# ross39/new_bloom_filter_repo

Hardware: AMD Instinct MI355X
Metric: Mpixels/s Bloom insert+query, 1080p residuals (higher is better)
Workload: dtype u64

## Files before the change

new_bloom_filter_repo_amd/csrc/rbf_api.hip:

```cpp
#include "rbf_host.h"
#include "rbf_kernels_noise.h"
#include "rbf_kernels_pack.h"
#include "rbf_rice_host.h"

#include <cmath>

struct MaskArgs {
    const void *frames; FrameLayout l; uint32_t nframes;
    int32_t thr_floor; const int32_t *thr_floors;
    void *masks; uint64_t mask_stride; uint64_t *ones;
    uint32_t channels;
};

static int launch_finish_ones(rbf_ctx *ctx, uint64_t *ones_dev, uint32_t pairs, uint64_t *host_block, uint64_t token,
                              void *clear_a, size_t bytes_a, void *clear_b, size_t bytes_b)
{
    if (clear_a && (((uintptr_t)clear_a | bytes_a) & 15)) { HIP_TRY(hipMemsetAsync(clear_a, 0, bytes_a, ctx->stream)); clear_a = nullptr; bytes_a = 0; }
    if (clear_b && (((uintptr_t)clear_b | bytes_b) & 15)) { HIP_TRY(hipMemsetAsync(clear_b, 0, bytes_b, ctx->stream)); clear_b = nullptr; bytes_b = 0; }
    const uint64_t quads = bytes_a / 16 + bytes_b / 16;
    uint32_t blocks = (uint32_t)((quads + 256 * 4 - 1) / (256 * 4));
    if (blocks < 1) blocks = 1;
    if (blocks > 1024) blocks = 1024;
    hipLaunchKernelGGL(k_finish_ones, dim3(blocks), dim3(256), 0, ctx->stream, ctx->ones_acc.p, ones_dev, pairs, host_block, token,
                       (uint4 *)clear_a, (uint64_t)(bytes_a / 16), (uint4 *)clear_b, (uint64_t)(bytes_b / 16));
// ... 228 lines not shown
}

struct QueryFlags {
    bool image_ready = false;
    bool table_for_next = false;
    bool quiet_passthrough = false;
};

static uint4 *table_to_rewrite(rbf_ctx *ctx, uint64_t n, const Seeds &sd)
{
    const SharedHashTable *sh = ctx->hash_shared;
    if (!sh || sh->n != n || !same_seeds(sh->seeds, sd) || ctx->knobs.no_hash_table || ctx->knobs.no_table_rewrite) return nullptr;
    std::lock_guard<std::mutex> lk(g_hash_mu);
    return sh->refs == 1 ? ctx->hash_tab : nullptr;
}

static int launch_query(rbf_ctx *ctx, const Plan &pl, const BloomBatch &b, const FrameTable &tab, const QueryFlags &flags)
{
    const uint32_t nframes = b.nframes;
    const Seeds sd = to_dev(*b.seeds);
    const uint32_t *filters = (const uint32_t *)b.filters;
    uint64_t stride_words = b.filter_stride / 4;
    if (pl.reads_probe_image()) {
        if (int r = ctx->qimage.reserve((size_t)nframes * pl.image_stride_words * 4)) return r;
        if (!flags.image_ready) {
            const uint32_t bx = (pl.image_stride_words + WG_THREADS - 1) / WG_THREADS;
            hipLaunchKernelGGL(k_probe_image, dim3(bx, nframes), dim3(WG_THREADS), 0, ctx->stream, filters, stride_words, ctx->qimage.p,
                               (uint64_t)pl.image_stride_words);
        }
        filters = ctx->qimage.p;
        stride_words = pl.image_stride_words;
    }
    const uint32_t lds_waves = (uint32_t)((pl.nseg + QL_WAVES - 1) / QL_WAVES);
    uint32_t nactive; uint64_t empty[2];
    LaunchTimer t(ctx, RBF_K_QUERY);
    if (pl.query == QueryKind::LdsTiledF64) {
        const FrameTable stab = query_table_s64(tab, nframes, &nactive, empty);
        if (flags.quiet_passthrough) empty[0] = empty[1] = 0;
        int mode = 0;
        for (uint32_t f = 0; f < nframes; ++f) {
            if (!tab.f[f].m) continue;
            if (tab.f[f].floor_k > 2) mode = 2;
            else if (tab.f[f].floor_k == 0 && mode < 1) mode = 1;
        }
        auto qkern = mode == 2 ? k_query_s64t<2> : mode == 1 ? k_query_s64t<1> : k_query_s64t<0>;
        if (int r = allow_big_lds((const void *)qkern)) return r;
        hipLaunchKernelGGL(qkern, dim3(lds_waves), dim3(QL_THREADS), s64t_lds_bytes(pl.query_tile_words), ctx->stream, b.n, nactive, stab, sd,
                           filters, stride_words, pl.query_tile_words, ctx->seg_cnt.p, pl.nseg, ctx->pass_words.p, empty[0], empty[1]);
    } else if (pl.reads_probe_image()) {
        uint4 *table_out = flags.table_for_next ? table_to_rewrite(ctx, b.n, sd) : nullptr;
        U64Classes cls;
        const FrameTable utab = query_table_u64(tab, nframes, &nactive, &cls, empty);
        if (flags.quiet_passthrough) empty[0] = empty[1] = 0;
        const bool wide = cls.n[3] + cls.n[4] > 0;
        auto kern64 = wide ? k_query_u64w : k_query_u64;
        if (int r = allow_big_lds((const void *)kern64)) return r;
        hipLaunchKernelGGL(kern64, dim3(lds_waves), dim3(QL_THREADS), pl.query_lds_bytes + u64_geo_bytes(nactive), ctx->stream, b.n, nactive,
                           utab, cls, sd, filters, stride_words, pl.fwords_max, ctx->seg_cnt.p, pl.nseg, ctx->pass_words.p, table_out, empty[0],
                           empty[1]);
    } else if (pl.query == QueryKind::LdsWhole) {
        auto kern = pl.double_buffer ? (pl.small_m ? k_query_lds<true, true> : k_query_lds<true, false>)
                                     : (pl.small_m ? k_query_lds<false, true> : k_query_lds<false, false>);
        if (int r = allow_big_lds((const void *)kern)) return r;
        hipLaunchKernelGGL(kern, dim3(lds_waves), dim3(QL_THREADS), pl.query_lds_bytes, ctx->stream, b.n, nframes, tab, sd, filters, stride_words,
                           pl.fwords_max, ctx->seg_cnt.p, pl.nseg, ctx->pass_words.p);
    } else if (pl.query == QueryKind::LdsTiled) {
        auto kern = pl.small_m ? k_query_tiled<true> : k_query_tiled<false>;
        if (int r = allow_big_lds((const void *)kern)) return r;
        hipLaunchKernelGGL(kern, dim3(lds_waves), dim3(QL_THREADS), pl.query_lds_bytes, ctx->stream, b.n, nframes, tab, sd, filters, stride_words,
                           pl.query_tile_words, ctx->seg_cnt.p, pl.nseg, ctx->pass_words.p);
    } else {
        const uint64_t bx = (pl.nseg + WG_WAVES - 1) / WG_WAVES;
        hipLaunchKernelGGL(k_query, dim3((uint32_t)bx, nframes), dim3(WG_THREADS), 0, ctx->stream, b.n, tab, sd, filters, stride_words,
                           ctx->seg_cnt.p, pl.nseg, ctx->pass_words.p);
    }
    return RBF_OK;
}

static int launch_insert_positions(rbf_ctx *ctx, const BloomBatch &b, const FrameTable &itab, const Seeds &sd, bool hashed_positions)
{
    HIP_TRY(hipMemsetAsync(ctx->ins_counters.p, 0, (size_t)b.nframes * 4, ctx->stream));
    const uint64_t groups = (((b.n + 7) >> 3) + IT_STEP_BYTES - 1) / IT_STEP_BYTES;
    uint64_t S1 = (uint64_t)ctx->cus * 4 / (b.nframes ? b.nframes : 1);
    if (S1 > groups / (IP_WAVES * 4)) S1 = groups / (IP_WAVES * 4);
    S1 &= ~7ull;
    if (S1 < 1) S1 = 1;
    if (int r = allow_big_lds((const void *)k_insert_records)) return r;
    LaunchTimer t(ctx, RBF_K_INSERT);
    auto pkern = hashed_positions ? k_insert_positions<true> : k_insert_positions<false>;
    hipLaunchKernelGGL(pkern, dim3((uint32_t)S1, b.nframes), dim3(IP_THREADS), 0, ctx->stream, (const uint8_t *)b.masks, b.mask_stride, b.n, itab,
                       hashed_positions ? nullptr : (const uint4 *)ctx->hash_tab, sd, ctx->ins_records.p, ctx->ins_counters.p);
    return RBF_OK;
}

static bool settle_hash_table(rbf_ctx *ctx, const Plan &pl, const BloomBatch &b, const Seeds &sd)
{
    const bool table_too_big = hash_table_bytes(b.n) > HASH_TABLE_CACHE_BYTES;
    if (table_too_big || (pl.insert_two_phase && ctx->knobs.hash_positions)) {
        if (ctx->hash_shared && (ctx->hash_shared->n != b.n || !same_seeds(ctx->hash_shared->seeds, *b.seeds))) hash_table_release(ctx);
        return true;
    }
    bool built = false;
    if (!hash_table_acquire(ctx, b.n, *b.seeds, &built)) return true;
    if (ctx->knobs.hash_rebuild && !built) launch_hash_table(ctx, b.n, sd, ctx->hash_tab);
    return false;
}

static int insert_fast(rbf_ctx *ctx, const Plan &pl, const BloomBatch &b, const FrameTable &tab, const uint64_t *ones_host, bool stream_once,
                       uint32_t *image)
{
    const uint32_t nframes = b.nframes;
    const Seeds sd = to_dev(*b.seeds);
// ... 1002 lines not shown
```

new_bloom_filter_repo_amd/csrc/rbf_device.h:

```cpp
#pragma once
#include <hip/hip_runtime.h>
#include <stdint.h>

namespace rbf {

constexpr uint64_t P1 = 0x9E3779B185EBCA87ULL;
constexpr uint64_t P2 = 0xC2B2AE3D27D4EB4FULL;
constexpr uint64_t P3 = 0x165667B19E3779F9ULL;
constexpr uint64_t P4 = 0x85EBCA77C2B2AE63ULL;
constexpr uint64_t P5 = 0x27D4EB2F165667C5ULL;

constexpr int WAVE = 64;

struct FrameDev {
    uint32_t m;
    uint32_t floor_k;
    uint64_t T;
    uint64_t M;
};

struct Seeds { uint64_t h1, h2, act; };

constexpr int MAX_BATCH = 128;
struct FrameTable { FrameDev f[MAX_BATCH]; };
// ... 32 lines not shown
    return k;
}

__device__ __forceinline__ uint64_t xxh64_key(const DecKey &k, uint64_t seed)
{
    uint64_t h = seed + P5 + (uint64_t)k.len;
    uint64_t rest;
    uint32_t cnt;
    if (k.len >= 8) {
        uint64_t k1 = k.lo * P2;
        k1 = rotl64(k1, 31) * P1;
        h ^= k1;
        h = rotl64(h, 27) * P1 + P4;
        rest = k.hi; cnt = k.len - 8;
    } else if (k.len >= 4) {
        h ^= (uint64_t)(uint32_t)k.lo * P1;
        h = rotl64(h, 23) * P2 + P3;
        rest = k.lo >> 32; cnt = k.len - 4;
    } else {
        rest = k.lo; cnt = k.len;
    }
    for (uint32_t t = 0; t < cnt; ++t) {
        h ^= (rest & 0xFFu) * P5;
        h = rotl64(h, 11) * P1;
        rest >>= 8;
    }
    h ^= h >> 33; h *= P2;
    h ^= h >> 29; h *= P3;
    h ^= h >> 32;
    return h;
}

struct Hash3 { uint64_t h1, h2, ha; };

template <int LEN>
__device__ __forceinline__ uint64_t xxh64_digits(const uint32_t (&d)[LEN], uint64_t seed)
{
    static_assert(LEN >= 5 && LEN <= 7, "4-byte round + 1..3 byte rounds");
    uint64_t h = seed + P5 + (uint64_t)LEN;
    const uint32_t w = 0x30303030u + d[0] + (d[1] << 8) + (d[2] << 16) + (d[3] << 24);
    h ^= (uint64_t)w * P1;
    h = rotl64(h, 23) * P2 + P3;
#pragma unroll
    for (int t = 4; t < LEN; ++t) {
        h ^= (uint64_t)(0x30u + d[t]) * P5;
        h = rotl64(h, 11) * P1;
    }
    h ^= h >> 33; h *= P2;
    h ^= h >> 29; h *= P3;
    h ^= h >> 32;
    return h;
}

template <int LEN>
__device__ __forceinline__ Hash3 hash3_fixed(uint32_t v, const Seeds &s)
{
    constexpr uint32_t P10[8] = {1u, 10u, 100u, 1000u, 10000u, 100000u, 1000000u, 10000000u};
    uint32_t q[LEN + 1];
#pragma unroll
    for (int k = 0; k <= LEN; ++k) q[k] = k < LEN ? v / P10[k] : 0u;
    uint32_t d[LEN];
#pragma unroll
    for (int k = 0; k < LEN; ++k) d[LEN - 1 - k] = q[k] - 10u * q[k + 1];
    Hash3 r;
    r.h1 = xxh64_digits<LEN>(d, s.h1);
    r.h2 = xxh64_digits<LEN>(d, s.h2);
    r.ha = xxh64_digits<LEN>(d, s.act);
    return r;
}

__device__ __forceinline__ Hash3 hash3_generic(uint32_t v, const Seeds &s)
{
    const DecKey key = make_key(v);
    Hash3 r;
    r.h1 = xxh64_key(key, s.h1);
    r.h2 = xxh64_key(key, s.h2);
    r.ha = xxh64_key(key, s.act);
    return r;
}

__device__ __forceinline__ Hash3 hash3_index(uint32_t v, bool active, const Seeds &s)
{
    const bool in7 = v >= 1000000u && v < 10000000u;
    const bool in6 = v >= 100000u && v < 1000000u;
    const bool in5 = v >= 10000u && v < 100000u;
    if (__all(!active || in7)) return hash3_fixed<7>(active ? v : 1000000u, s);
    if (__all(!active || in6)) return hash3_fixed<6>(active ? v : 100000u, s);
    if (__all(!active || in5)) return hash3_fixed<5>(active ? v : 10000u, s);
    return hash3_generic(active ? v : 0u, s);
}

struct Prefix3 { uint64_t h1, h2, ha; };

template <int LEN>
__device__ __forceinline__ Prefix3 hash3_decade_prefix(uint32_t decade , const Seeds &s)
{
    static_assert(LEN >= 5 && LEN <= 7, "key = decade digits + one more character");
    constexpr uint32_t P10[7] = {1u, 10u, 100u, 1000u, 10000u, 100000u, 1000000u};
    uint32_t q[LEN];
#pragma unroll
    for (int k = 0; k < LEN; ++k) q[k] = k < LEN - 1 ? decade / P10[k] : 0u;
    uint32_t d[LEN - 1];
#pragma unroll
    for (int k = 0; k < LEN - 1; ++k) d[LEN - 2 - k] = q[k] - 10u * q[k + 1];
    const uint64_t lane4 = (uint64_t)(0x30303030u + d[0] + (d[1] << 8) + (d[2] << 16) + (d[3] << 24)) * P1;
    uint64_t h[3] = {s.h1 + P5 + (uint64_t)LEN, s.h2 + P5 + (uint64_t)LEN, s.act + P5 + (uint64_t)LEN};
#pragma unroll
    for (int c = 0; c < 3; ++c) h[c] = rotl64(h[c] ^ lane4, 23) * P2 + P3;
#pragma unroll
    for (int t = 4; t < LEN - 1; ++t) {
        const uint64_t term = (uint64_t)(0x30u + d[t]) * P5;
#pragma unroll
        for (int c = 0; c < 3; ++c) h[c] = rotl64(h[c] ^ term, 11) * P1;
    }
    return Prefix3{h[0], h[1], h[2]};
}

__device__ __forceinline__ uint64_t xxh64_last_byte(uint64_t h, uint64_t term )
{
    h = rotl64(h ^ term, 11) * P1;
    h ^= h >> 33; h *= P2;
    h ^= h >> 29; h *= P3;
    h ^= h >> 32;
    return h;
}

template <int LEN>
__device__ __forceinline__ void hash3_run8_fixed(uint32_t v0, const Seeds &s, uint64_t (&h1)[8], uint64_t (&h2)[8], uint64_t (&ha)[8])
{
    const uint32_t decade = v0 / 10u, r0 = v0 - decade * 10u;
    const Prefix3 a = hash3_decade_prefix<LEN>(decade, s);
    const Prefix3 b = hash3_decade_prefix<LEN>(decade + 1u, s);
#pragma unroll
    for (int j = 0; j < 8; ++j) {
        const uint32_t t = r0 + (uint32_t)j;
        const bool in_b = t >= 10u;
        const uint64_t term = (uint64_t)(0x30u + (in_b ? t - 10u : t)) * P5;
        h1[j] = xxh64_last_byte(in_b ? b.h1 : a.h1, term);
        h2[j] = xxh64_last_byte(in_b ? b.h2 : a.h2, term);
        ha[j] = xxh64_last_byte(in_b ? b.ha : a.ha, term);
    }
}

__device__ __forceinline__ bool hash3_run8(uint32_t v0, uint32_t valid, const Seeds &s, uint64_t (&h1)[8], uint64_t (&h2)[8], uint64_t (&ha)[8])
{
    const bool active = valid != 0u;
    const uint32_t v7 = v0 + 7u;
    const bool in7 = v0 >= 1000000u && v7 < 10000000u;
    const bool in6 = v0 >= 100000u && v7 < 1000000u;
    const bool in5 = v0 >= 10000u && v7 < 100000u;
    if (__all(!active || in7)) { hash3_run8_fixed<7>(active ? v0 : 1000000u, s, h1, h2, ha); return true; }
    if (__all(!active || in6)) { hash3_run8_fixed<6>(active ? v0 : 100000u, s, h1, h2, ha); return true; }
    if (__all(!active || in5)) { hash3_run8_fixed<5>(active ? v0 : 10000u, s, h1, h2, ha); return true; }
    return false;
}

template <int LEN>
__device__ __forceinline__ void hash3_run4_fixed(uint32_t v0, const Seeds &s, uint64_t (&h1)[4], uint64_t (&h2)[4], uint64_t (&ha)[4])
{
    const uint32_t decade = v0 / 10u, r0 = v0 - decade * 10u;
    const Prefix3 a = hash3_decade_prefix<LEN>(decade, s);
    const Prefix3 b = hash3_decade_prefix<LEN>(decade + 1u, s);
#pragma unroll
    for (int j = 0; j < 4; ++j) {
        const uint32_t t = r0 + (uint32_t)j;
        const bool in_b = t >= 10u;
        const uint64_t term = (uint64_t)(0x30u + (in_b ? t - 10u : t)) * P5;
        h1[j] = xxh64_last_byte(in_b ? b.h1 : a.h1, term);
        h2[j] = xxh64_last_byte(in_b ? b.h2 : a.h2, term);
        ha[j] = xxh64_last_byte(in_b ? b.ha : a.ha, term);
    }
}

__device__ __forceinline__ bool hash3_run4(uint32_t v0, uint32_t valid, const Seeds &s, uint64_t (&h1)[4], uint64_t (&h2)[4], uint64_t (&ha)[4])
{
    const bool active = valid != 0u;
    const uint32_t v3 = v0 + 3u;
    const bool in7 = v0 >= 1000000u && v3 < 10000000u;
    const bool in6 = v0 >= 100000u && v3 < 1000000u;
    const bool in5 = v0 >= 10000u && v3 < 100000u;
    if (__all(!active || in7)) { hash3_run4_fixed<7>(active ? v0 : 1000000u, s, h1, h2, ha); return true; }
    if (__all(!active || in6)) { hash3_run4_fixed<6>(active ? v0 : 100000u, s, h1, h2, ha); return true; }
    if (__all(!active || in5)) { hash3_run4_fixed<5>(active ? v0 : 10000u, s, h1, h2, ha); return true; }
    return false;
}

__device__ __forceinline__ uint32_t mod_m(uint64_t h, uint32_t m, uint64_t M)
{
    if (m == 1u) return 0u;
    const uint64_t q = __umul64hi(h, M);
    uint64_t r = h - q * (uint64_t)m;
    if (r >= m) r -= m;
    return (uint32_t)r;
}

struct Probe {
    uint32_t pos;
    uint32_t step;
    bool extra;
};

__device__ __forceinline__ Probe make_probe(uint32_t index, const FrameDev &f, const Seeds &s)
{
    const DecKey key = make_key(index);
    Probe p;
    p.pos = mod_m(xxh64_key(key, s.h1), f.m, f.M);
// ... 13 lines not shown
```

new_bloom_filter_repo_amd/csrc/rbf_kernels_lds.h:

```cpp
#pragma once
#include "rbf_kernels.h"

namespace rbf {

typedef uint32_t nt_u32x4 __attribute__((ext_vector_type(4)));
__device__ __forceinline__ void store_stream(uint4 *p, uint4 v) { const nt_u32x4 x = {v.x, v.y, v.z, v.w}; __builtin_nontemporal_store(x, reinterpret_cast<nt_u32x4 *>(p)); }
__device__ __forceinline__ uint4 load_stream(const uint4 *p) { const nt_u32x4 x = __builtin_nontemporal_load(reinterpret_cast<const nt_u32x4 *>(p)); return make_uint4(x.x, x.y, x.z, x.w); }

constexpr int QL_THREADS = 1024;
constexpr int QL_WAVES = QL_THREADS / WAVE;
constexpr int QL_P = 8;
constexpr int QL_SEG_PIXELS = QL_P * WAVE;

constexpr int IL_THREADS = 1024;
constexpr int IL_WAVES = IL_THREADS / WAVE;
constexpr int IL_QUEUE = 64 + 512;

__device__ __forceinline__ void wave_lds_fence()
{
    __builtin_amdgcn_fence(__ATOMIC_RELEASE, "wavefront");
    __builtin_amdgcn_wave_barrier();
    __builtin_amdgcn_fence(__ATOMIC_ACQUIRE, "wavefront");
}

// ... 625 lines not shown
    if (lane == WAVE - 1) wsum[wave] = incl;
    __syncthreads();
    uint32_t o = start32 + incl - c;
#pragma unroll
    for (int k = 0; k < WG_WAVES; ++k)
        if ((uint32_t)k < wave) o += wsum[k];
    if (w >= nwords) return;
    uint64_t out = 0;
    if (c) {
        const uint32_t d0 = o >> 5, dl = (o + c - 1u) >> 5, r = o & 31u;
        const uint64_t x0 = d0 < witness_stride_words32 ? flip_bytes32(wit[d0]) : 0u;
        const uint64_t x1 = (d0 + 1 <= dl && d0 + 1 < witness_stride_words32) ? flip_bytes32(wit[d0 + 1]) : 0u;
        const uint64_t x2 = (d0 + 2 <= dl && d0 + 2 < witness_stride_words32) ? flip_bytes32(wit[d0 + 2]) : 0u;
        uint64_t win = (x0 | (x1 << 32)) >> r;
        win |= r ? x2 << (64u - r) : 0ull;
        out = (uint64_t)pdep32_lut(lut, (uint32_t)win, p_lo) | ((uint64_t)pdep32_lut(lut, (uint32_t)(win >> c_lo), p_hi) << 32);
    }
    masks[(uint64_t)f * mask_stride_words64 + w] = flip_bytes64(out);
}

}

namespace rbf {

template <typename SAMPLE, int PIXEL_BYTES>
struct LanePixels {
    static constexpr int DW = 16 * PIXEL_BYTES / 4;
    uint32_t d[DW];
    template <bool NT>
    __device__ __forceinline__ void load(const uint8_t *p)
    {
        typedef uint32_t u32x4 __attribute__((ext_vector_type(4)));
        const u32x4 *q = reinterpret_cast<const u32x4 *>(p);
#pragma unroll
        for (int i = 0; i < DW / 4; ++i) {
            const u32x4 v = NT ? __builtin_nontemporal_load(q + i) : q[i];
            d[4 * i] = v.x; d[4 * i + 1] = v.y; d[4 * i + 2] = v.z; d[4 * i + 3] = v.w;
        }
    }
    __device__ __forceinline__ uint32_t luma(int k) const
    {
        const int byte = k * PIXEL_BYTES;
        const uint32_t w = d[byte >> 2];
        if (sizeof(SAMPLE) == 1) return (w >> (8 * (byte & 3))) & 0xFFu;
        return (w >> (8 * (byte & 3))) & 0xFFFFu;
    }
};

template <typename SAMPLE, int PIXEL_BYTES>
__device__ __forceinline__ uint32_t lane_bits_thr0(const LanePixels<SAMPLE, PIXEL_BYTES> &a, const LanePixels<SAMPLE, PIXEL_BYTES> &b, uint32_t one2, uint32_t &count_src)
{
    uint32_t bits = 0;
    if (sizeof(SAMPLE) == 1) {
        constexpr int shift_of_group[4] = {4, 0, 12, 8};
#pragma unroll
        for (int g = 0; g < 4; ++g) {
            uint32_t z;
            if (PIXEL_BYTES == 1) z = a.d[g] ^ b.d[g];
            else {
                const uint32_t x0 = a.d[3 * g] ^ b.d[3 * g], x1 = a.d[3 * g + 1] ^ b.d[3 * g + 1], x2 = a.d[3 * g + 2] ^ b.d[3 * g + 2];
                const uint32_t y = __builtin_amdgcn_perm(x1, x0, 0x00060300u);
                z = __builtin_amdgcn_perm(x2, y, 0x05020100u);
            }
            const uint32_t f = (((z & 0x7F7F7F7Fu) + 0x7F7F7F7Fu) | z) & 0x80808080u;
            bits |= (((f >> 7) * 0x08040201u) >> 24) << shift_of_group[g];
        }
        count_src = bits;
    } else if (PIXEL_BYTES == 2) {
        const uint32_t k7 = 0x7FFF7FFFu;
        uint32_t acc = 0;
#pragma unroll
        for (int s = 0; s < 8; ++s) {
            const int j = s ^ 4;
            const uint32_t t = (a.d[j] ^ b.d[j]) & k7;
            uint32_t g;
            asm("v_pk_min_u16 %0, %1, %2" : "=v"(g) : "v"(t), "v"(one2));
            acc = (acc << 2) | g;
        }
        bits = (acc >> 16) | (acc << 1);
        count_src = acc;
    } else {
        typedef unsigned short h2 __attribute__((ext_vector_type(2)));
#pragma unroll
        for (int j = 0; j < 8; ++j) {
            const h2 t0 = __builtin_bit_cast(h2, a.d[3 * j]) - __builtin_bit_cast(h2, b.d[3 * j]);
            const h2 t1 = __builtin_bit_cast(h2, a.d[3 * j + 1]) - __builtin_bit_cast(h2, b.d[3 * j + 1]);
            const uint32_t d = (__builtin_bit_cast(uint32_t, t0) & 0x0000FFFFu) | (__builtin_bit_cast(uint32_t, t1) & 0xFFFF0000u);
            const uint32_t f = ((d & 0x7FFF7FFFu) + 0x7FFF7FFFu) & 0x80008000u;
            const uint32_t two = ((f >> 14) & 2u) | (f >> 31);
            bits |= two << (((2 * j + 1) ^ 7));
        }
        count_src = bits;
    }
    return bits;
}

template <typename SAMPLE, int PIXEL_BYTES>
__device__ __forceinline__ uint32_t lane_bits_any(const LanePixels<SAMPLE, PIXEL_BYTES> &a, const LanePixels<SAMPLE, PIXEL_BYTES> &b, uint32_t one2, uint32_t &count_src)
{
    static_assert(PIXEL_BYTES == 3 || PIXEL_BYTES == 4 || PIXEL_BYTES == 6 || PIXEL_BYTES == 8, "all-channel masks: 3 or 4 samples of 1 or 2 bytes");
    uint32_t bits = 0;
    if (PIXEL_BYTES == 3) {
        constexpr int shift_of_group[4] = {4, 0, 12, 8};
#pragma unroll
        for (int g = 0; g < 4; ++g) {
            const uint32_t x0 = a.d[3 * g] ^ b.d[3 * g], x1 = a.d[3 * g + 1] ^ b.d[3 * g + 1], x2 = a.d[3 * g + 2] ^ b.d[3 * g + 2];
            const uint32_t s0 = __builtin_amdgcn_perm(x2, __builtin_amdgcn_perm(x1, x0, 0x00060300u), 0x05020100u);
            const uint32_t s1 = __builtin_amdgcn_perm(x2, __builtin_amdgcn_perm(x1, x0, 0x00070401u), 0x06020100u);
            const uint32_t s2 = __builtin_amdgcn_perm(x2, __builtin_amdgcn_perm(x1, x0, 0x00000502u), 0x07040100u);
            const uint32_t z = s0 | s1 | s2;
            const uint32_t f = (((z & 0x7F7F7F7Fu) + 0x7F7F7F7Fu) | z) & 0x80808080u;
            bits |= (((f >> 7) * 0x08040201u) >> 24) << shift_of_group[g];
        }
        count_src = bits;
    } else if (PIXEL_BYTES == 4 || PIXEL_BYTES == 8) {
        constexpr int DPP = PIXEL_BYTES / 4;
#pragma unroll
        for (int k = 0; k < 16; ++k) {
            uint32_t t = a.d[DPP * k] ^ b.d[DPP * k];
// ... 100 lines not shown
```

new_bloom_filter_repo_amd/csrc/rbf_kernels_u64.h:

```cpp
#pragma once
#include "rbf_kernels_s64.h"
#include <algorithm>
#include <cstring>
#include <type_traits>

namespace rbf {

constexpr uint32_t U64_REC_BYTES = 32;
__host__ __device__ constexpr uint32_t u64_geo_bytes(uint32_t nactive) { return (nactive + 1u) * U64_REC_BYTES; }
constexpr int U64_CLASSES = 6;

struct U64Classes { uint32_t n[U64_CLASSES]; };

__host__ inline FrameTable query_table_u64(const FrameTable &tab, uint32_t nframes, uint32_t *nactive, U64Classes *cls, uint64_t (&empty)[2])
{
    FrameTable q;
    memset(&q, 0, sizeof q);
    memset(cls, 0, sizeof *cls);
    empty[0] = empty[1] = 0;
    uint64_t sorted[MAX_BATCH];
    uint32_t coded = 0;
    for (uint32_t f = 0; f < nframes; ++f) {
        if (tab.f[f].m) sorted[coded++] = tab.f[f].T;
        else empty[f >> 6] |= 1ull << (f & 63);
// ... 18 lines not shown
    return q;
}

template <bool ON>
struct RowDmaC {
    const uint8_t *image;
    uint32_t src;
    uint32_t dst_m0;
    uint64_t mask[5];
    bool full;

    __device__ __forceinline__ void issue() const
    {
        uint32_t keep; uint64_t keepx;
        if (full) {
            asm volatile("s_mov_b32 %0, m0\n\t"
                         "s_mov_b32 m0, %1\n\t"
                         "s_nop 0\n\t"
                         "global_load_lds_dwordx4 %2, %3 offset:-2048\n\t"
                         "global_load_lds_dwordx4 %2, %3 offset:-1024\n\t"
                         "global_load_lds_dwordx4 %2, %3\n\t"
                         "global_load_lds_dwordx4 %2, %3 offset:1024\n\t"
                         "global_load_lds_dwordx4 %2, %3 offset:2048\n\t"
                         "s_mov_b32 m0, %0"
                         : "=&s"(keep) : "s"(dst_m0), "v"(src), "s"(image) : "memory");
            return;
        }
        asm volatile("s_mov_b32 %0, m0\n\t"
                     "s_mov_b64 %1, exec\n\t"
                     "s_mov_b32 m0, %2\n\t"
                     "s_mov_b64 exec, %5\n\t"
                     "global_load_lds_dwordx4 %3, %4 offset:-2048\n\t"
                     "s_mov_b64 exec, %6\n\t"
                     "global_load_lds_dwordx4 %3, %4 offset:-1024\n\t"
                     "s_mov_b64 exec, %7\n\t"
                     "global_load_lds_dwordx4 %3, %4\n\t"
                     "s_mov_b64 exec, %8\n\t"
                     "global_load_lds_dwordx4 %3, %4 offset:1024\n\t"
                     "s_mov_b64 exec, %9\n\t"
                     "global_load_lds_dwordx4 %3, %4 offset:2048\n\t"
                     "s_mov_b64 exec, %1\n\t"
                     "s_mov_b32 m0, %0"
                     : "=&s"(keep), "=&s"(keepx)
                     : "s"(dst_m0), "v"(src), "s"(image), "s"(mask[0]), "s"(mask[1]), "s"(mask[2]), "s"(mask[3]), "s"(mask[4])
                     : "memory");
    }
    __device__ __forceinline__ void at(int g)
    {
        if (ON && g == 0) issue();
    }
};


template <bool WIDE>
__device__ __forceinline__ void query_u64_body(
    uint64_t n, uint32_t nactive, const FrameTable &tab, const U64Classes &cls, Seeds seeds,
    const uint32_t *__restrict__ image, uint64_t image_stride_words32, uint32_t fwords_max,
    uint32_t *__restrict__ seg_cnt, uint64_t nseg, uint64_t *__restrict__ pass_words,
    uint4 *__restrict__ table_out, uint64_t empty_lo, uint64_t empty_hi)
{
    extern __shared__ __attribute__((aligned(16))) uint32_t lds[];
    const uint32_t bufwords = ((fwords_max + 3u) & ~3u) + 4u;
    const uint32_t safe_pos = ((fwords_max + 3u) & ~3u) << 5;
    const uint32_t lane = threadIdx.x & 63u, wave = __builtin_amdgcn_readfirstlane(threadIdx.x >> 6);
    const uint32_t seg = blockIdx.x * QL_WAVES + wave;
    const bool live = seg < nseg;
    if (threadIdx.x < 8u) lds[(threadIdx.x >> 2) * bufwords + (bufwords - 4u) + (threadIdx.x & 3u)] = 0u;
    uint4 *geo = reinterpret_cast<uint4 *>(lds + 2u * bufwords);
    uint64_t *tl = reinterpret_cast<uint64_t *>(lds + bufwords);
    FrameDev fd_mine{};
    if (threadIdx.x < 2u * MAX_BATCH) fd_mine = tab.f[threadIdx.x < nactive ? threadIdx.x : 0u];

    static_assert(QL_P == 8, "a lane's verdicts fill one byte");
    double hd1[QL_P], hd2[QL_P];
    uint32_t hl1[QL_P], hl2[QL_P];
    uint32_t rank_lo = 0, rank_hi = 0;
    uint32_t validmask = 0;
    const uint64_t i0 = (uint64_t)seg * QL_SEG_PIXELS + (uint64_t)lane * QL_P;
    {
        uint64_t h1[QL_P], h2[QL_P], ha[QL_P];
#pragma unroll
        for (int it = 0; it < QL_P; ++it) {
            h1[it] = 0; h2[it] = 0; ha[it] = ~0ull;
            if (live && i0 + it < n) validmask |= 1u << it;
        }
        if (!hash3_run8((uint32_t)i0, validmask, seeds, h1, h2, ha)) {
#pragma unroll
            for (int it = 0; it < QL_P; ++it) {
                const bool act = (validmask >> it) & 1u;
                const Hash3 h = hash3_index((uint32_t)(i0 + it), act, seeds);
                h1[it] = h.h1; h2[it] = h.h2; ha[it] = h.ha;
            }
        }
#pragma unroll
        for (int it = 0; it < QL_P; ++it) {
            hd1[it] = (double)h1[it]; hl1[it] = (uint32_t)h1[it];
            hd2[it] = (double)h2[it]; hl2[it] = (uint32_t)h2[it];
        }
        if (table_out && live) hash_table_store8(table_out, n, seg, lane, h1, h2, ha);
        if (threadIdx.x < 2u * MAX_BATCH) {
            const uint32_t t = threadIdx.x;
            tl[t] = t < nactive ? fd_mine.T : ~0ull;
            if (t < nactive) {
                const uint32_t f = fd_mine.floor_k >> 16;
                const uint32_t row = (uint32_t)((uint64_t)f * image_stride_words32 * 4u);
                const uint32_t out_row = (uint32_t)((uint64_t)f * nseg);
                geo[2u * t] = make_uint4(fd_mine.m, (fd_mine.floor_k >> 8) & 0xFFu, (uint32_t)fd_mine.M, (uint32_t)(fd_mine.M >> 32));
                uint32_t *w = reinterpret_cast<uint32_t *>(geo);
                if (t) w[8u * (t - 1u) + 4u] = row;
                if (t + 1u == nactive) w[8u * t + 4u] = row;
                if (t == 0u) w[8u * nactive + 4u] = row;
                w[8u * t + 6u] = fd_mine.floor_k & 0xFFu;
                w[8u * (t + 1u) + 7u] = out_row;
            }
        }
        __syncthreads();
        uint32_t top = 1;
        while (2u * top <= nactive) top *= 2u;
        top = __builtin_amdgcn_readfirstlane(top);
        uint32_t r[QL_P];
#pragma unroll
        for (int it = 0; it < QL_P; ++it) r[it] = 0;
        for (uint32_t step = top; step; step >>= 1) {
#pragma unroll
            for (int it = 0; it < QL_P; ++it) {
                const uint64_t t = tl[r[it] + step - 1u];
                r[it] |= t <= ha[it] ? step : 0u;
            }
        }
        rank_lo = r[0] | (r[1] << 8) | (r[2] << 16) | (r[3] << 24);
        rank_hi = r[4] | (r[5] << 8) | (r[6] << 16) | (r[7] << 24);
    }
    const bool whole_wave = __builtin_amdgcn_readfirstlane((uint32_t)__all(validmask == 0xFFu)) != 0u;
    uint8_t *pass_bytes = reinterpret_cast<uint8_t *>(pass_words);

    for (uint32_t half = 0; half < 2; ++half) {
        uint64_t bits = half ? empty_hi : empty_lo;
        while (bits) {
            const uint32_t g = half * 64u + (uint32_t)__builtin_ctzll(bits);
            bits &= bits - 1;
            if (live && lane == 0) seg_cnt[(uint64_t)g * nseg + seg] = 0;
            if (live) pass_bytes[((uint64_t)g * nseg + seg) * (QL_SEG_PIXELS / 8) + lane] = 0;
        }
    }
    if (nactive == 0) return;

    const uint32_t lds0 = __builtin_amdgcn_readfirstlane(lds_addr_of(lds));
    const uint32_t pitch_bytes = (uint32_t)image_stride_words32 * 4u;
    const uint32_t off0 = wave * 5120u + lane * 16u;
    RowDmaC<true> dm;
    dm.image = reinterpret_cast<const uint8_t *>(image);
#pragma unroll
    for (int i = 0; i < 5; ++i) dm.mask[i] = __ballot(off0 + (uint32_t)i * 1024u + 16u <= pitch_bytes);
    dm.full = dm.mask[4] == ~0ull;
    const uint32_t off0b = off0 + 2048u, wave_dst = wave * 5120u + 2048u;
    const uint32_t buf_sum = lds0 + lds0 + bufwords * 4u;
    uint32_t fbase = vgpr_copy(lds0);
    {
        const uint32_t *w = reinterpret_cast<const uint32_t *>(geo);
        dm.src = w[8u * nactive + 4u] + off0 + 2048u;
        dm.dst_m0 = lds0 + wave * 5120u + 2048u;
        dm.at(0);
    }
    const uint32_t safe_v = vgpr_copy(safe_pos);
    const uint32_t seg_lane = seg * (QL_SEG_PIXELS / 8) + lane;
    uint32_t cnt2 = 0;
    uint32_t row_prev = 0, row_prev2 = 0;
    uint32_t out_row = 0;
    uint32_t out_pb = 0;
    bool out_pending = false, have_two = false;

    auto flush = [&]() {
        if (!out_pending) return;
        if (live) pass_bytes[(out_row << 6) + seg_lane] = (uint8_t)out_pb;
        {
            cnt2 = __builtin_amdgcn_alignbit(__popc(out_pb), cnt2, 16);
            row_prev2 = row_prev; row_prev = out_row;
            if (have_two) {
                const uint32_t tot = wave_sum_to_lane63(cnt2);
                if (live && lane == 63u) {
                    seg_cnt[row_prev2 + seg] = tot & 0xFFFFu;
                    seg_cnt[row_prev + seg] = tot >> 16;
                }
            }
            have_two = !have_two;
        }
    };

    uint32_t j = 0;
    auto frames = [&](auto fk_tag, uint32_t count) {
        constexpr int FK = decltype(fk_tag)::value;
        const uint32_t end = j + count;
        for (; j < end; ++j) {
            const uint4 ga = geo[2u * j], gb = geo[2u * j + 1u];
            const uint32_t m_v = ga.x, c_v = ga.y;
            const double ninv = __builtin_bit_cast(double, ((uint64_t)(uint32_t)__builtin_amdgcn_readfirstlane(ga.w) << 32) | (uint32_t)__builtin_amdgcn_readfirstlane(ga.z));
            uint32_t x[4] = {0, 0, 0, 0};
            const bool rows = FK > 0 && whole_wave;
            if (rows) rows_reduce4(0, hd1, hl1, hd2, hl2, m_v, ninv, x);
            dm.src = gb.x + off0b;
            dm.dst_m0 = (uint32_t)__builtin_amdgcn_readfirstlane(buf_sum - fbase) + wave_dst;
            dma_wait_all();
            out_row = (uint32_t)__builtin_amdgcn_readfirstlane(gb.w);
            __syncthreads();
            uint32_t pbf = 0;
            if (rows) {
                if constexpr (FK > 0) frame_pass_rows<FK, (FK < 5), true>(hd1, hl1, hd2, hl2, rank_lo, rank_hi, c_v, fbase, safe_v, m_v, ninv, x, pbf, dm, flush);
            } else {
                flush();
                const uint32_t fk = FK > 0 ? (uint32_t)FK : (uint32_t)__builtin_amdgcn_readfirstlane(gb.z);
                frame_pass_plain(hd1, hl1, hd2, hl2, rank_lo, rank_hi, c_v, validmask, fbase, safe_v, m_v, ninv, fk, pbf, dm);
            }
            out_pb = ~pbf & 0xFFu; out_pending = true;
            fbase = buf_sum - fbase;
        }
    };
    frames(std::integral_constant<int, 1>{}, cls.n[0]);
    frames(std::integral_constant<int, 2>{}, cls.n[1]);
    frames(std::integral_constant<int, 3>{}, cls.n[2]);
    if constexpr (WIDE) {
        frames(std::integral_constant<int, 4>{}, cls.n[3]);
        frames(std::integral_constant<int, 5>{}, cls.n[4]);
    }
    frames(std::integral_constant<int, 0>{}, cls.n[5] + (WIDE ? 0u : cls.n[3] + cls.n[4]));
    out_row = (uint32_t)__builtin_amdgcn_readfirstlane(reinterpret_cast<const uint32_t *>(geo)[8u * nactive + 7u]);
    flush();
    if (have_two) {
        const uint32_t tot = wave_sum_to_lane63(cnt2);
        if (live && lane == 63u) seg_cnt[row_prev + seg] = tot >> 16;
    }
}

#define RBF_U64_PARAMS uint64_t n, uint32_t nactive, const FrameTable tab, const U64Classes cls, Seeds seeds, const uint32_t *__restrict__ image, uint64_t image_stride_words32, \
    uint32_t fwords_max, uint32_t *__restrict__ seg_cnt, uint64_t nseg, uint64_t *__restrict__ pass_words, uint4 *__restrict__ table_out, uint64_t empty_lo, uint64_t empty_hi
#define RBF_U64_ARGS n, nactive, tab, cls, seeds, image, image_stride_words32, fwords_max, seg_cnt, nseg, pass_words, table_out, empty_lo, empty_hi
__attribute__((amdgpu_num_vgpr(60))) __global__ __launch_bounds__(QL_THREADS) void k_query_u64(RBF_U64_PARAMS) { query_u64_body<false>(RBF_U64_ARGS); }
__global__ __launch_bounds__(QL_THREADS) void k_query_u64w(RBF_U64_PARAMS) { query_u64_body<true>(RBF_U64_ARGS); }
#undef RBF_U64_PARAMS
#undef RBF_U64_ARGS

}
```

new_bloom_filter_repo_amd/csrc/rbf_plan.h:

```cpp
#pragma once
#include "../../include/rbf.h"
#include "rbf_kernels_i64.h"
#include "rbf_kernels_u64.h"

#include <algorithm>
#include <cstring>

using namespace rbf;

static int fail(int code, const char *fmt, ...);

struct Knobs {
    bool force_generic = false;
    bool single_buffer = false;
    bool force_generic_mask_bits = false;
    bool barrett_only = false;
    bool hash_rebuild = false;
    bool no_hash_table = false;
    bool no_two_phase = false;
    bool hash_positions = false;
    bool no_table_rewrite = false;
    bool no_fused_finish = false;
    uint32_t mask_chunks = 0;
    uint32_t tile_words = 0;
    uint32_t insert_slices = 0;
    void set_flags(int on)
    {
        force_generic = on & 1;
        single_buffer = on & 2;
        force_generic_mask_bits = on & 4;
        barrett_only = on & 8;
        hash_rebuild = on & 16;
        no_hash_table = on & 32;
        no_two_phase = on & 128;
        mask_chunks = (uint32_t)(on >> 8) & 0x1F;
        hash_positions = on & (1 << 14);
        no_table_rewrite = on & (1 << 15);
        tile_words = ((uint32_t)on >> 16) << 6;
    }
    bool fp64_kernels() const { return !force_generic && !barrett_only && !single_buffer; }
};

static inline FrameDev frame_dev(const rbf_filter_params &p)
{
    return FrameDev{p.m, p.floor_k, p.threshold, p.m >= 2 ? (uint64_t)((((unsigned __int128)1) << 64) / p.m) : 0};
}

static int fill_table(const rbf_filter_params *params, uint32_t count, FrameTable *tab)
{
    memset(tab, 0, sizeof *tab);
    for (uint32_t f = 0; f < count; ++f) {
        if (params[f].floor_k > 64) return fail(RBF_ERANGE, "frame %u: floor_k %u > 64", f, params[f].floor_k);
        tab->f[f] = frame_dev(params[f]);
    }
    return RBF_OK;
}

static FrameTable query_table_s64(const FrameTable &tab, uint32_t nframes, uint32_t *nactive, uint64_t (&empty)[2])
{
    FrameTable q;
    memset(&q, 0, sizeof q);
    empty[0] = empty[1] = 0;
    uint64_t sorted[MAX_BATCH];
    uint32_t coded = 0;
    for (uint32_t f = 0; f < nframes; ++f) {
        if (tab.f[f].m) sorted[coded++] = tab.f[f].T;
        else empty[f >> 6] |= 1ull << (f & 63);
    }
    std::sort(sorted, sorted + coded);
    uint32_t j = 0;
    for (uint32_t f = 0; f < nframes; ++f) {
        if (!tab.f[f].m) continue;
        const double ninv = -1.0 / (double)tab.f[f].m;
        const uint32_t below = (uint32_t)(std::lower_bound(sorted, sorted + coded, tab.f[f].T) - sorted);
        q.f[j].m = tab.f[f].m;
        memcpy(&q.f[j].M, &ninv, 8);
        q.f[j].floor_k = tab.f[f].floor_k | (below << 8) | (f << 16);
        q.f[j].T = sorted[j];
        ++j;
    }
    *nactive = coded;
    return q;
}

constexpr size_t LDS_LIMIT = 160 * 1024;
constexpr size_t HASH_TABLE_CACHE_BYTES = (size_t)96 << 20;
// ... 159 lines not shown
```

Before: 556,400.

## Use cached 16-bit activation tags from shared hash table in u64 query

When a shared hash table with matching seeds and size already exists, the u64 query kernel loads precomputed 16-bit activation-hash tags and ranks pixels against 16-bit threshold prefixes. It skips computing the third (activation) xxh64 hash and reads the full activation hash from the table only on tag ties. This trades hashing arithmetic for an extra global load per lane plus an occasional tie fallback. The change also repacks byte-mask nibbles with a single perm and moves the DMA source setup to read the first frame's floor directly.

```diff
diff --git a/new_bloom_filter_repo_amd/csrc/rbf_api.hip b/new_bloom_filter_repo_amd/csrc/rbf_api.hip
--- a/new_bloom_filter_repo_amd/csrc/rbf_api.hip
+++ b/new_bloom_filter_repo_amd/csrc/rbf_api.hip
@@ -304,12 +304,17 @@
         U64Classes cls;
         const FrameTable utab = query_table_u64(tab, nframes, &nactive, &cls, empty);
         if (flags.quiet_passthrough) empty[0] = empty[1] = 0;
+        const uint4 *table_in = nullptr;
+        if (flags.table_for_next && !table_out && !ctx->knobs.no_hash_table && !ctx->knobs.no_query_tags && pl.fwords_max >= 1024u) {
+            const SharedHashTable *sh = ctx->hash_shared;
+            if (sh && sh->n == b.n && same_seeds(sh->seeds, sd)) table_in = ctx->hash_tab;
+        }
         const bool wide = cls.n[3] + cls.n[4] > 0;
-        auto kern64 = wide ? k_query_u64w : k_query_u64;
+        auto kern64 = table_in ? (wide ? k_query_u64wt : k_query_u64t) : (wide ? k_query_u64w : k_query_u64);
         if (int r = allow_big_lds((const void *)kern64)) return r;
         hipLaunchKernelGGL(kern64, dim3(lds_waves), dim3(QL_THREADS), pl.query_lds_bytes + u64_geo_bytes(nactive), ctx->stream, b.n, nactive,
                            utab, cls, sd, filters, stride_words, pl.fwords_max, ctx->seg_cnt.p, pl.nseg, ctx->pass_words.p, table_out, empty[0],
-                           empty[1]);
+                           empty[1], table_in);
     } else if (pl.query == QueryKind::LdsWhole) {
         auto kern = pl.double_buffer ? (pl.small_m ? k_query_lds<true, true> : k_query_lds<true, false>)
                                      : (pl.small_m ? k_query_lds<false, true> : k_query_lds<false, false>);
diff --git a/new_bloom_filter_repo_amd/csrc/rbf_device.h b/new_bloom_filter_repo_amd/csrc/rbf_device.h
--- a/new_bloom_filter_repo_amd/csrc/rbf_device.h
+++ b/new_bloom_filter_repo_amd/csrc/rbf_device.h
@@ -108,7 +108,7 @@
     return h;
 }
 
-template <int LEN>
+template <int LEN, bool ACT = true>
 __device__ __forceinline__ Hash3 hash3_fixed(uint32_t v, const Seeds &s)
 {
     constexpr uint32_t P10[8] = {1u, 10u, 100u, 1000u, 10000u, 100000u, 1000000u, 10000000u};
@@ -121,38 +121,41 @@
     Hash3 r;
     r.h1 = xxh64_digits<LEN>(d, s.h1);
     r.h2 = xxh64_digits<LEN>(d, s.h2);
-    r.ha = xxh64_digits<LEN>(d, s.act);
+    r.ha = ACT ? xxh64_digits<LEN>(d, s.act) : 0ull;
     return r;
 }
 
+template <bool ACT = true>
 __device__ __forceinline__ Hash3 hash3_generic(uint32_t v, const Seeds &s)
 {
     const DecKey key = make_key(v);
     Hash3 r;
     r.h1 = xxh64_key(key, s.h1);
     r.h2 = xxh64_key(key, s.h2);
-    r.ha = xxh64_key(key, s.act);
+    r.ha = ACT ? xxh64_key(key, s.act) : 0ull;
     return r;
 }
 
+template <bool ACT = true>
 __device__ __forceinline__ Hash3 hash3_index(uint32_t v, bool active, const Seeds &s)
 {
     const bool in7 = v >= 1000000u && v < 10000000u;
     const bool in6 = v >= 100000u && v < 1000000u;
     const bool in5 = v >= 10000u && v < 100000u;
-    if (__all(!active || in7)) return hash3_fixed<7>(active ? v : 1000000u, s);
-    if (__all(!active || in6)) return hash3_fixed<6>(active ? v : 100000u, s);
-    if (__all(!active || in5)) return hash3_fixed<5>(active ? v : 10000u, s);
-    return hash3_generic(active ? v : 0u, s);
+    if (__all(!active || in7)) return hash3_fixed<7, ACT>(active ? v : 1000000u, s);
+    if (__all(!active || in6)) return hash3_fixed<6, ACT>(active ? v : 100000u, s);
+    if (__all(!active || in5)) return hash3_fixed<5, ACT>(active ? v : 10000u, s);
+    return hash3_generic<ACT>(active ? v : 0u, s);
 }
 
 struct Prefix3 { uint64_t h1, h2, ha; };
 
-template <int LEN>
+template <int LEN, bool ACT = true>
 __device__ __forceinline__ Prefix3 hash3_decade_prefix(uint32_t decade , const Seeds &s)
 {
     static_assert(LEN >= 5 && LEN <= 7, "key = decade digits + one more character");
     constexpr uint32_t P10[7] = {1u, 10u, 100u, 1000u, 10000u, 100000u, 1000000u};
+    constexpr int NH = ACT ? 3 : 2;
     uint32_t q[LEN];
 #pragma unroll
     for (int k = 0; k < LEN; ++k) q[k] = k < LEN - 1 ? decade / P10[k] : 0u;
@@ -162,12 +165,12 @@
     const uint64_t lane4 = (uint64_t)(0x30303030u + d[0] + (d[1] << 8) + (d[2] << 16) + (d[3] << 24)) * P1;
     uint64_t h[3] = {s.h1 + P5 + (uint64_t)LEN, s.h2 + P5 + (uint64_t)LEN, s.act + P5 + (uint64_t)LEN};
 #pragma unroll
-    for (int c = 0; c < 3; ++c) h[c] = rotl64(h[c] ^ lane4, 23) * P2 + P3;
+    for (int c = 0; c < NH; ++c) h[c] = rotl64(h[c] ^ lane4, 23) * P2 + P3;
 #pragma unroll
     for (int t = 4; t < LEN - 1; ++t) {
         const uint64_t term = (uint64_t)(0x30u + d[t]) * P5;
 #pragma unroll
-        for (int c = 0; c < 3; ++c) h[c] = rotl64(h[c] ^ term, 11) * P1;
+        for (int c = 0; c < NH; ++c) h[c] = rotl64(h[c] ^ term, 11) * P1;
     }
     return Prefix3{h[0], h[1], h[2]};
 }
@@ -181,12 +184,12 @@
     return h;
 }
 
-template <int LEN>
+template <int LEN, bool ACT = true>
 __device__ __forceinline__ void hash3_run8_fixed(uint32_t v0, const Seeds &s, uint64_t (&h1)[8], uint64_t (&h2)[8], uint64_t (&ha)[8])
 {
     const uint32_t decade = v0 / 10u, r0 = v0 - decade * 10u;
-    const Prefix3 a = hash3_decade_prefix<LEN>(decade, s);
-    const Prefix3 b = hash3_decade_prefix<LEN>(decade + 1u, s);
+    const Prefix3 a = hash3_decade_prefix<LEN, ACT>(decade, s);
+    const Prefix3 b = hash3_decade_prefix<LEN, ACT>(decade + 1u, s);
 #pragma unroll
     for (int j = 0; j < 8; ++j) {
         const uint32_t t = r0 + (uint32_t)j;
@@ -194,10 +197,11 @@
         const uint64_t term = (uint64_t)(0x30u + (in_b ? t - 10u : t)) * P5;
         h1[j] = xxh64_last_byte(in_b ? b.h1 : a.h1, term);
         h2[j] = xxh64_last_byte(in_b ? b.h2 : a.h2, term);
-        ha[j] = xxh64_last_byte(in_b ? b.ha : a.ha, term);
-    }
-}
-
+        if constexpr (ACT) ha[j] = xxh64_last_byte(in_b ? b.ha : a.ha, term);
+    }
+}
+
+template <bool ACT = true>
 __device__ __forceinline__ bool hash3_run8(uint32_t v0, uint32_t valid, const Seeds &s, uint64_t (&h1)[8], uint64_t (&h2)[8], uint64_t (&ha)[8])
 {
     const bool active = valid != 0u;
@@ -205,9 +209,9 @@
     const bool in7 = v0 >= 1000000u && v7 < 10000000u;
     const bool in6 = v0 >= 100000u && v7 < 1000000u;
     const bool in5 = v0 >= 10000u && v7 < 100000u;
-    if (__all(!active || in7)) { hash3_run8_fixed<7>(active ? v0 : 1000000u, s, h1, h2, ha); return true; }
-    if (__all(!active || in6)) { hash3_run8_fixed<6>(active ? v0 : 100000u, s, h1, h2, ha); return true; }
-    if (__all(!active || in5)) { hash3_run8_fixed<5>(active ? v0 : 10000u, s, h1, h2, ha); return true; }
+    if (__all(!active || in7)) { hash3_run8_fixed<7, ACT>(active ? v0 : 1000000u, s, h1, h2, ha); return true; }
+    if (__all(!active || in6)) { hash3_run8_fixed<6, ACT>(active ? v0 : 100000u, s, h1, h2, ha); return true; }
+    if (__all(!active || in5)) { hash3_run8_fixed<5, ACT>(active ? v0 : 10000u, s, h1, h2, ha); return true; }
     return false;
 }
 
diff --git a/new_bloom_filter_repo_amd/csrc/rbf_kernels_lds.h b/new_bloom_filter_repo_amd/csrc/rbf_kernels_lds.h
--- a/new_bloom_filter_repo_amd/csrc/rbf_kernels_lds.h
+++ b/new_bloom_filter_repo_amd/csrc/rbf_kernels_lds.h
@@ -701,7 +701,7 @@
 {
     uint32_t bits = 0;
     if (sizeof(SAMPLE) == 1) {
-        constexpr int shift_of_group[4] = {4, 0, 12, 8};
+        uint32_t nib[4];
 #pragma unroll
         for (int g = 0; g < 4; ++g) {
             uint32_t z;
@@ -712,8 +712,9 @@
                 z = __builtin_amdgcn_perm(x2, y, 0x05020100u);
             }
             const uint32_t f = (((z & 0x7F7F7F7Fu) + 0x7F7F7F7Fu) | z) & 0x80808080u;
-            bits |= (((f >> 7) * 0x08040201u) >> 24) << shift_of_group[g];
-        }
+            nib[g] = (f >> 7) * ((g & 1) ? 0x08040201u : 0x80402010u);
+        }
+        bits = __builtin_amdgcn_perm(nib[2] | nib[3], nib[0] | nib[1], 0x0c0c0703u);
         count_src = bits;
     } else if (PIXEL_BYTES == 2) {
         const uint32_t k7 = 0x7FFF7FFFu;
diff --git a/new_bloom_filter_repo_amd/csrc/rbf_kernels_u64.h b/new_bloom_filter_repo_amd/csrc/rbf_kernels_u64.h
--- a/new_bloom_filter_repo_amd/csrc/rbf_kernels_u64.h
+++ b/new_bloom_filter_repo_amd/csrc/rbf_kernels_u64.h
@@ -94,12 +94,12 @@
 };
 
 
-template <bool WIDE>
+template <bool WIDE, bool TAGS>
 __device__ __forceinline__ void query_u64_body(
     uint64_t n, uint32_t nactive, const FrameTable &tab, const U64Classes &cls, Seeds seeds,
     const uint32_t *__restrict__ image, uint64_t image_stride_words32, uint32_t fwords_max,
     uint32_t *__restrict__ seg_cnt, uint64_t nseg, uint64_t *__restrict__ pass_words,
-    uint4 *__restrict__ table_out, uint64_t empty_lo, uint64_t empty_hi)
+    uint4 *__restrict__ table_out, uint64_t empty_lo, uint64_t empty_hi, const uint4 *__restrict__ table_in)
 {
     extern __shared__ __attribute__((aligned(16))) uint32_t lds[];
     const uint32_t bufwords = ((fwords_max + 3u) & ~3u) + 4u;
@@ -110,6 +110,10 @@
     if (threadIdx.x < 8u) lds[(threadIdx.x >> 2) * bufwords + (bufwords - 4u) + (threadIdx.x & 3u)] = 0u;
     uint4 *geo = reinterpret_cast<uint4 *>(lds + 2u * bufwords);
     uint64_t *tl = reinterpret_cast<uint64_t *>(lds + bufwords);
+    uint4 tags = make_uint4(0, 0, 0, 0);
+    if constexpr (TAGS)
+        if (live) tags = *reinterpret_cast<const uint4 *>(HashTable(const_cast<uint4 *>(table_in), n).tag + (uint64_t)seg * QL_SEG_PIXELS + lane * QL_P);
+    uint32_t *tt = reinterpret_cast<uint32_t *>(tl + 2u * MAX_BATCH);
     FrameDev fd_mine{};
     if (threadIdx.x < 2u * MAX_BATCH) fd_mine = tab.f[threadIdx.x < nactive ? threadIdx.x : 0u];
 
@@ -126,12 +130,13 @@
             h1[it] = 0; h2[it] = 0; ha[it] = ~0ull;
             if (live && i0 + it < n) validmask |= 1u << it;
         }
-        if (!hash3_run8((uint32_t)i0, validmask, seeds, h1, h2, ha)) {
+        if (!hash3_run8<!TAGS>((uint32_t)i0, validmask, seeds, h1, h2, ha)) {
 #pragma unroll
             for (int it = 0; it < QL_P; ++it) {
                 const bool act = (validmask >> it) & 1u;
-                const Hash3 h = hash3_index((uint32_t)(i0 + it), act, seeds);
-                h1[it] = h.h1; h2[it] = h.h2; ha[it] = h.ha;
+                const Hash3 h = hash3_index<!TAGS>((uint32_t)(i0 + it), act, seeds);
+                h1[it] = h.h1; h2[it] = h.h2;
+                if constexpr (!TAGS) ha[it] = h.ha;
             }
         }
 #pragma unroll
@@ -139,10 +144,15 @@
             hd1[it] = (double)h1[it]; hl1[it] = (uint32_t)h1[it];
             hd2[it] = (double)h2[it]; hl2[it] = (uint32_t)h2[it];
         }
-        if (table_out && live) hash_table_store8(table_out, n, seg, lane, h1, h2, ha);
+        if constexpr (!TAGS)
+            if (table_out && live) hash_table_store8(table_out, n, seg, lane, h1, h2, ha);
         if (threadIdx.x < 2u * MAX_BATCH) {
             const uint32_t t = threadIdx.x;
             tl[t] = t < nactive ? fd_mine.T : ~0ull;
+            if constexpr (TAGS) {
+                tt[1u + t] = t < nactive ? (uint32_t)(fd_mine.T >> 48) : ~0u;
+                if (t == 0u) tt[0] = ~0u;
+            }
             if (t < nactive) {
                 const uint32_t f = fd_mine.floor_k >> 16;
                 const uint32_t row = (uint32_t)((uint64_t)f * image_stride_words32 * 4u);
@@ -151,7 +161,6 @@
                 uint32_t *w = reinterpret_cast<uint32_t *>(geo);
                 if (t) w[8u * (t - 1u) + 4u] = row;
                 if (t + 1u == nactive) w[8u * t + 4u] = row;
-                if (t == 0u) w[8u * nactive + 4u] = row;
                 w[8u * t + 6u] = fd_mine.floor_k & 0xFFu;
                 w[8u * (t + 1u) + 7u] = out_row;
             }
@@ -163,15 +172,42 @@
         uint32_t r[QL_P];
 #pragma unroll
         for (int it = 0; it < QL_P; ++it) r[it] = 0;
-        for (uint32_t step = top; step; step >>= 1) {
-#pragma unroll
-            for (int it = 0; it < QL_P; ++it) {
-                const uint64_t t = tl[r[it] + step - 1u];
-                r[it] |= t <= ha[it] ? step : 0u;
-            }
+        uint32_t ties = 0;
+        if constexpr (!TAGS) {
+            for (uint32_t step = top; step; step >>= 1) {
+#pragma unroll
+                for (int it = 0; it < QL_P; ++it) {
+                    const uint64_t t = tl[r[it] + step - 1u];
+                    r[it] |= t <= ha[it] ? step : 0u;
+                }
+            }
+        } else {
+            const uint32_t tag[QL_P] = {tags.x & 0xFFFFu, tags.x >> 16, tags.y & 0xFFFFu, tags.y >> 16, tags.z & 0xFFFFu, tags.z >> 16, tags.w & 0xFFFFu, tags.w >> 16};
+            for (uint32_t step = top; step; step >>= 1) {
+#pragma unroll
+                for (int it = 0; it < QL_P; ++it) r[it] |= tt[r[it] + step] <= tag[it] ? step : 0u;
+            }
+#pragma unroll
+            for (int it = 0; it < QL_P; ++it) ties |= tt[r[it]] == tag[it] ? 1u << it : 0u;
+            ties &= validmask;
         }
         rank_lo = r[0] | (r[1] << 8) | (r[2] << 16) | (r[3] << 24);
         rank_hi = r[4] | (r[5] << 8) | (r[6] << 16) | (r[7] << 24);
+        if constexpr (TAGS) {
+            if (ties) {
+                const HashTable ht(const_cast<uint4 *>(table_in), n);
+                do {
+                    const uint32_t it = (uint32_t)__builtin_ctz(ties);
+                    ties &= ties - 1u;
+                    const uint64_t hact = ht.act[hash_table_slot((uint32_t)i0 + it)];
+                    uint32_t rr = 0;
+                    for (uint32_t step = top; step; step >>= 1) rr |= tl[rr + step - 1u] <= hact ? step : 0u;
+                    const uint32_t sh = (it & 3u) * 8u;
+                    if (it < 4u) rank_lo = (rank_lo & ~(0xFFu << sh)) | (rr << sh);
+                    else rank_hi = (rank_hi & ~(0xFFu << sh)) | (rr << sh);
+                } while (ties);
+            }
+        }
     }
     const bool whole_wave = __builtin_amdgcn_readfirstlane((uint32_t)__all(validmask == 0xFFu)) != 0u;
     uint8_t *pass_bytes = reinterpret_cast<uint8_t *>(pass_words);
@@ -195,15 +231,12 @@
 #pragma unroll
     for (int i = 0; i < 5; ++i) dm.mask[i] = __ballot(off0 + (uint32_t)i * 1024u + 16u <= pitch_bytes);
     dm.full = dm.mask[4] == ~0ull;
+    dm.src = (tab.f[0].floor_k >> 16) * pitch_bytes + off0 + 2048u;
+    dm.dst_m0 = lds0 + wave * 5120u + 2048u;
+    dm.at(0);
     const uint32_t off0b = off0 + 2048u, wave_dst = wave * 5120u + 2048u;
     const uint32_t buf_sum = lds0 + lds0 + bufwords * 4u;
     uint32_t fbase = vgpr_copy(lds0);
-    {
-        const uint32_t *w = reinterpret_cast<const uint32_t *>(geo);
-        dm.src = w[8u * nactive + 4u] + off0 + 2048u;
-        dm.dst_m0 = lds0 + wave * 5120u + 2048u;
-        dm.at(0);
-    }
     const uint32_t safe_v = vgpr_copy(safe_pos);
     const uint32_t seg_lane = seg * (QL_SEG_PIXELS / 8) + lane;
     uint32_t cnt2 = 0;
@@ -274,10 +307,13 @@
 }
 
 #define RBF_U64_PARAMS uint64_t n, uint32_t nactive, const FrameTable tab, const U64Classes cls, Seeds seeds, const uint32_t *__restrict__ image, uint64_t image_stride_words32, \
-    uint32_t fwords_max, uint32_t *__restrict__ seg_cnt, uint64_t nseg, uint64_t *__restrict__ pass_words, uint4 *__restrict__ table_out, uint64_t empty_lo, uint64_t empty_hi
-#define RBF_U64_ARGS n, nactive, tab, cls, seeds, image, image_stride_words32, fwords_max, seg_cnt, nseg, pass_words, table_out, empty_lo, empty_hi
-__attribute__((amdgpu_num_vgpr(60))) __global__ __launch_bounds__(QL_THREADS) void k_query_u64(RBF_U64_PARAMS) { query_u64_body<false>(RBF_U64_ARGS); }
-__global__ __launch_bounds__(QL_THREADS) void k_query_u64w(RBF_U64_PARAMS) { query_u64_body<true>(RBF_U64_ARGS); }
+    uint32_t fwords_max, uint32_t *__restrict__ seg_cnt, uint64_t nseg, uint64_t *__restrict__ pass_words, uint4 *__restrict__ table_out, uint64_t empty_lo, uint64_t empty_hi, \
+    const uint4 *__restrict__ table_in
+#define RBF_U64_ARGS n, nactive, tab, cls, seeds, image, image_stride_words32, fwords_max, seg_cnt, nseg, pass_words, table_out, empty_lo, empty_hi, table_in
+__attribute__((amdgpu_num_vgpr(60))) __global__ __launch_bounds__(QL_THREADS) void k_query_u64(RBF_U64_PARAMS) { query_u64_body<false, false>(RBF_U64_ARGS); }
+__global__ __launch_bounds__(QL_THREADS) void k_query_u64w(RBF_U64_PARAMS) { query_u64_body<true, false>(RBF_U64_ARGS); }
+__attribute__((amdgpu_num_vgpr(60))) __global__ __launch_bounds__(QL_THREADS) void k_query_u64t(RBF_U64_PARAMS) { query_u64_body<false, true>(RBF_U64_ARGS); }
+__global__ __launch_bounds__(QL_THREADS) void k_query_u64wt(RBF_U64_PARAMS) { query_u64_body<true, true>(RBF_U64_ARGS); }
 #undef RBF_U64_PARAMS
 #undef RBF_U64_ARGS
 
diff --git a/new_bloom_filter_repo_amd/csrc/rbf_plan.h b/new_bloom_filter_repo_amd/csrc/rbf_plan.h
--- a/new_bloom_filter_repo_amd/csrc/rbf_plan.h
+++ b/new_bloom_filter_repo_amd/csrc/rbf_plan.h
@@ -20,6 +20,7 @@
     bool no_two_phase = false;
     bool hash_positions = false;
     bool no_table_rewrite = false;
+    bool no_query_tags = false;
     bool no_fused_finish = false;
     uint32_t mask_chunks = 0;
     uint32_t tile_words = 0;
@@ -32,6 +33,7 @@
         barrett_only = on & 8;
         hash_rebuild = on & 16;
         no_hash_table = on & 32;
+        no_query_tags = on & 64;
         no_two_phase = on & 128;
         mask_chunks = (uint32_t)(on >> 8) & 0x1F;
         hash_positions = on & (1 << 14);
```

New measurement: 568,000, median of 6. +2.1%, better.
